# acaelles97/DeVIS

Measured on NVIDIA B200. Metric: temporal_msda_fwd_bwd_layer_clips_per_sec, higher is better.
Workload: dtype f32

## Files before the change

### devis_b200/csrc/msda_bwd.cuh

```cuda
#pragma once
#include "msda_common.cuh"

#ifndef DEVIS_BWD_MIN_BLOCKS
#define DEVIS_BWD_MIN_BLOCKS 3
#endif

namespace devis {

template <class SlotSrc>
struct BwdArgs {
    const void *value;
    const void *grad_out;
    void *grad_value;
    DetScale det;
    Segment seg[2];
    int n_seg;
    int n_slots_total;
    SlotSrc src;
    OpDims d;
    const int *q_perm;
};

template <int LPG>
__device__ __forceinline__ void reduce_scatter_taps(float (&d)[LPG][4], int j, float (&r)[4])
{
#pragma unroll
    for (int half = LPG / 2; half >= 1; half >>= 1) {
        const bool upper = (j & half) != 0;
#pragma unroll
        for (int t = 0; t < half; ++t) {
#pragma unroll
            for (int c = 0; c < 4; ++c) {
                const float send = upper ? d[t][c] : d[t + half][c];
                const float keep = upper ? d[t + half][c] : d[t][c];
                d[t][c] = keep + __shfl_xor_sync(0xffffffffu, send, half, LPG);
            }
        }
    }
#pragma unroll
    for (int c = 0; c < 4; ++c) r[c] = d[0][c];
}

template <bool BF16, int LPG, int QPG, class SlotSrc, bool HALF_ACC = false>
__global__ void __launch_bounds__(256, DEVIS_BWD_MIN_BLOCKS) msda_bwd_kernel(const BwdArgs<SlotSrc> a)
{
    using X = TapExchange<LPG>;
    extern __shared__ int4 s_slot[];
    const int outer = blockIdx.y;
    build_slots(s_slot, a.src, a.d, outer, a.n_slots_total);
    float *xbuf = reinterpret_cast<float *>(s_slot + a.n_slots_total) + (threadIdx.x >> 5) * (2 * X::kWordsPerWarpBuf);

    const int M = a.d.M, Lq = a.d.Lq;
    const int j = threadIdx.x % LPG;
    const int g = (threadIdx.x & 31) / LPG;
    const int grp = threadIdx.x / LPG;
    const int QC = blockDim.x / LPG;
    const int qchunk = blockIdx.x / M, m = blockIdx.x - qchunk * M;
    const L2Policy pol = make_l2_policy();

    int q[QPG];
    bool qlive[QPG];
    float4 go[QPG];
#pragma unroll
    for (int i = 0; i < QPG; ++i) {
        const int qi = (qchunk * QPG + i) * QC + grp;
        qlive[i] = qi < Lq;
        q[i] = qlive[i] ? (a.q_perm ? a.q_perm[qi] : qi) : 0;
        go[i] = make_float4(0.f, 0.f, 0.f, 0.f);
        if (qlive[i]) {
            const size_t row = ((size_t)outer * Lq + q[i]) * M + m;
            go[i] = BF16 ? ldg_bf16x4(reinterpret_cast<const uint2 *>(a.grad_out) + row * LPG + j)
                         : ld_stream_f4(reinterpret_cast<const float4 *>(a.grad_out) + row * LPG + j, pol);
        }
    }

    constexpr unsigned kQuadBytes = BF16 ? 8u : 16u;
    const unsigned rowbytes = (unsigned)(M * LPG) * kQuadBytes;
    const char *vbase = reinterpret_cast<const char *>(a.value) + (size_t)(m * LPG + j) * kQuadBytes;
    asm volatile("" : "+l"(vbase));
    static_assert(!HALF_ACC || BF16, "bf16 accumulation needs bf16 value");
    constexpr unsigned kGvQuadBytes = HALF_ACC ? 8u : 16u;
    char *gvb = a.grad_value ? reinterpret_cast<char *>(a.grad_value) + (size_t)(m * LPG + j) * kGvQuadBytes : nullptr;
    constexpr unsigned kGvShift = (BF16 && !HALF_ACC) ? 1u : 0u;
    char *detb = a.det.acc ? reinterpret_cast<char *>(a.det.acc) + (size_t)(m * LPG) * 32u + (size_t)j * 8u : nullptr;
    const float det_sh = a.det.acc ? ldexpf(1.f, kDetFracBits - det_exponent(a.det.max_bits)) : 0.f;

    int slot_base = 0, parity = 0;
    for (int sg = 0; sg < a.n_seg; ++sg) {
        const int P = a.seg[sg].P, K = a.seg[sg].n_slots * P, pshift = pow2_shift(P);
        const float *loc = reinterpret_cast<const float *>(a.seg[sg].loc);
        const float *aw = reinterpret_cast<const float *>(a.seg[sg].aw);
        float *gloc = reinterpret_cast<float *>(a.seg[sg].grad_loc);
        float *gaw = reinterpret_cast<float *>(a.seg[sg].grad_aw);
        for (int k0 = 0; k0 < K; k0 += LPG) {
            const int k = k0 + j;
            const bool klive = k < K;
            const int4 sl = s_slot[slot_base + (klive ? div_p(k, P, pshift) : 0)];
#pragma unroll
            for (int i = 0; i < QPG; ++i) {
                const size_t row = ((size_t)outer * Lq + q[i]) * M + m;
                const bool live = klive && qlive[i];
                float2 xy = make_float2(0.f, 0.f);
                float w = 0.f;
                if (live) {
                    xy = ld_stream_f2(reinterpret_cast<const float2 *>(loc + row * K * 2) + k, pol);
                    w = ld_stream_f(aw + row * K + k, pol);
                }
                const TapGeom t = tap_geometry(xy.x, xy.y, sl, live);
                float *buf = xbuf + parity * X::kWordsPerWarpBuf;
                parity ^= 1;
                X::publish(buf, j, g, t, w, rowbytes);
                __syncwarp();

                const float4 gg = go[i];
                float dsum[LPG][4];
#pragma unroll
                for (int jj = 0; jj < LPG; ++jj) {
                    uint4 off;
                    float4 c;
                    X::fetch(buf, jj, g, off, c);
                    float4 v00, v01, v10, v11;
                    if (BF16) {
                        v00 = ldg_bf16x4(reinterpret_cast<const uint2 *>(vbase + off.x));
                        v01 = ldg_bf16x4(reinterpret_cast<const uint2 *>(vbase + off.y));
                        v10 = ldg_bf16x4(reinterpret_cast<const uint2 *>(vbase + off.z));
                        v11 = ldg_bf16x4(reinterpret_cast<const uint2 *>(vbase + off.w));
                    } else {
                        v00 = ldg_f4(reinterpret_cast<const float4 *>(vbase + off.x), pol);
                        v01 = ldg_f4(reinterpret_cast<const float4 *>(vbase + off.y), pol);
                        v10 = ldg_f4(reinterpret_cast<const float4 *>(vbase + off.z), pol);
                        v11 = ldg_f4(reinterpret_cast<const float4 *>(vbase + off.w), pol);
                    }
                    dsum[jj][0] = fmaf(v00.w, gg.w, fmaf(v00.z, gg.z, fmaf(v00.y, gg.y, v00.x * gg.x)));
                    dsum[jj][1] = fmaf(v01.w, gg.w, fmaf(v01.z, gg.z, fmaf(v01.y, gg.y, v01.x * gg.x)));
                    dsum[jj][2] = fmaf(v10.w, gg.w, fmaf(v10.z, gg.z, fmaf(v10.y, gg.y, v10.x * gg.x)));
                    dsum[jj][3] = fmaf(v11.w, gg.w, fmaf(v11.z, gg.z, fmaf(v11.y, gg.y, v11.x * gg.x)));
                    if (detb) {
                        if (c.x != 0.f) det_add4<LPG>(reinterpret_cast<long long *>(detb + ((size_t)off.x << (kGvShift + 1))), det_sh, c.x * gg.x, c.x * gg.y, c.x * gg.z, c.x * gg.w);
                        if (c.y != 0.f) det_add4<LPG>(reinterpret_cast<long long *>(detb + ((size_t)off.y << (kGvShift + 1))), det_sh, c.y * gg.x, c.y * gg.y, c.y * gg.z, c.y * gg.w);
                        if (c.z != 0.f) det_add4<LPG>(reinterpret_cast<long long *>(detb + ((size_t)off.z << (kGvShift + 1))), det_sh, c.z * gg.x, c.z * gg.y, c.z * gg.z, c.z * gg.w);
                        if (c.w != 0.f) det_add4<LPG>(reinterpret_cast<long long *>(detb + ((size_t)off.w << (kGvShift + 1))), det_sh, c.w * gg.x, c.w * gg.y, c.w * gg.z, c.w * gg.w);
                    } else if (gvb) {
                        if (c.x != 0.f) red_add_quad<HALF_ACC>(gvb + ((size_t)off.x << kGvShift), c.x * gg.x, c.x * gg.y, c.x * gg.z, c.x * gg.w, pol);
                        if (c.y != 0.f) red_add_quad<HALF_ACC>(gvb + ((size_t)off.y << kGvShift), c.y * gg.x, c.y * gg.y, c.y * gg.z, c.y * gg.w, pol);
                        if (c.z != 0.f) red_add_quad<HALF_ACC>(gvb + ((size_t)off.z << kGvShift), c.z * gg.x, c.z * gg.y, c.z * gg.z, c.z * gg.w, pol);
                        if (c.w != 0.f) red_add_quad<HALF_ACC>(gvb + ((size_t)off.w << kGvShift), c.w * gg.x, c.w * gg.y, c.w * gg.z, c.w * gg.w, pol);
                    }
                }

                float A[4];
                reduce_scatter_taps<LPG>(dsum, j, A);
                if (live) {
                    const bool hit = t.ok != 0u;
                    const float hh = (t.ok & 1u) ? t.hh : 0.f, lh = (t.ok & 2u) ? t.lh : 0.f;
                    const float hw = (t.ok & 4u) ? t.hw : 0.f, lw = (t.ok & 8u) ? t.lw : 0.f;
                    const float l_in = (t.ok & 4u) ? 1.f : 0.f, r_in = (t.ok & 8u) ? 1.f : 0.f;
                    const float t_in = (t.ok & 1u) ? 1.f : 0.f, b_in = (t.ok & 2u) ? 1.f : 0.f;
                    const float val = hh * (hw * A[0] + lw * A[1]) + lh * (hw * A[2] + lw * A[3]);
                    const float gx = hh * (r_in * A[1] - l_in * A[0]) + lh * (r_in * A[3] - l_in * A[2]);
                    const float gy = hw * (b_in * A[2] - t_in * A[0]) + lw * (b_in * A[3] - t_in * A[1]);
                    st_stream_f(gaw + row * K + k, hit ? val : 0.f, pol);
                    st_stream_f2(reinterpret_cast<float2 *>(gloc + row * K * 2) + k,
                                 hit ? make_float2((float)sl.y * gx * w, (float)sl.x * gy * w) : make_float2(0.f, 0.f), pol);
                }
            }
        }
        slot_base += a.seg[sg].n_slots;
    }
}

}
```

### devis_b200/csrc/msda_common.cuh

```cuda
#pragma once
#include <cuda_bf16.h>
#include <cuda_runtime.h>
#include <stdint.h>

namespace devis {

constexpr int kMaxLevels = 16;
constexpr int kMaxFrameTable = 2048;
constexpr int kMaxSlots = 1024;

struct Segment {
    const void *loc;
    const void *aw;
    void *grad_loc;
    void *grad_aw;
    int n_slots;
    int P;
};

struct DeviceLevels {
    const int64_t *shapes;
    const int64_t *lsi;
};

struct ClipTable {
    int H[kMaxLevels];
    int W[kMaxLevels];
    int lsi[kMaxLevels];
    int L;
    int Wt;
    uint8_t frame[kMaxFrameTable];
};

struct OpDims {
    int outer;
    int S;
    int M, D;
    int Lq;
};

__device__ __forceinline__ void build_slots(int4 *s_slot, const DeviceLevels &lv, const OpDims &d, int outer,
                                            int n_slots)
{
    for (int s = threadIdx.x; s < n_slots; s += blockDim.x) {
        const int H = (int)lv.shapes[2 * s], W = (int)lv.shapes[2 * s + 1];
        s_slot[s] = make_int4(H, W, outer * d.S + (int)lv.lsi[s], W * d.M);
    }
    __syncthreads();
}

__device__ __forceinline__ void build_slots(int4 *s_slot, const ClipTable &tb, const OpDims &d, int outer,
                                            int n_slots)
{
    for (int s = threadIdx.x; s < n_slots; s += blockDim.x) {
        int frame, l;
        if (s < tb.L) {
            frame = outer;
            l = s;
        } else {
            const int j = (s - tb.L) / tb.L;
            l = (s - tb.L) - j * tb.L;
            frame = tb.frame[outer * tb.Wt + j];
        }
        s_slot[s] = make_int4(tb.H[l], tb.W[l], frame * d.S + tb.lsi[l], tb.W[l] * d.M);
    }
    __syncthreads();
}

__device__ __forceinline__ int pow2_shift(int v) { return (v > 0 && (v & (v - 1)) == 0) ? __ffs(v) - 1 : -1; }
__device__ __forceinline__ int div_p(int k, int P, int pshift) { return pshift >= 0 ? (k >> pshift) : (k / P); }
__device__ __forceinline__ int mod_l(int s, int L, int lshift) { return lshift >= 0 ? (s & (L - 1)) : (s % L); }

struct TapGeom {
    float lh, lw, hh, hw;
    int rTL, rTR, rBL, rBR;
    int y0c, x0c;
    unsigned ok;
};

__device__ __forceinline__ TapGeom tap_geometry(float x, float y, const int4 slot, bool live)
{
    TapGeom g;
    const int H = slot.x, W = slot.y;
    const float h_im = __fadd_rn(__fmul_rn(y, (float)H), -0.5f);
    const float w_im = __fadd_rn(__fmul_rn(x, (float)W), -0.5f);
    const bool inb = live && h_im > -1.f && w_im > -1.f && h_im < (float)H && w_im < (float)W;
    const float hf = floorf(h_im), wf = floorf(w_im);
    const int h0 = inb ? (int)hf : 0, w0 = inb ? (int)wf : 0;
    g.lh = h_im - hf;
    g.lw = w_im - wf;
    g.hh = 1.f - g.lh;
    g.hw = 1.f - g.lw;
    g.ok = inb ? ((unsigned)(h0 >= 0) | ((unsigned)(h0 + 1 <= H - 1) << 1) | ((unsigned)(w0 >= 0) << 2) |
                  ((unsigned)(w0 + 1 <= W - 1) << 3))
               : 0u;
    const int h0c = max(h0, 0), h1c = min(h0 + 1, H - 1), w0c = max(w0, 0), w1c = min(w0 + 1, W - 1);
    const int top = slot.z + h0c * W, bot = slot.z + h1c * W;
    g.y0c = h0c;
    g.x0c = w0c;
    g.rTL = top + w0c;
    g.rTR = top + w1c;
    g.rBL = bot + w0c;
    g.rBR = bot + w1c;
    return g;
}

struct TapGeomV {
    float lh, lw, hh, hw;
    int rowv;
    unsigned live;
    unsigned ok;
};

__device__ __forceinline__ TapGeomV tap_geometry_v(float x, float y, const int4 slot, bool live)
{
    TapGeomV g;
    const int H = slot.x, W = slot.y;
    const float h_im = __fadd_rn(__fmul_rn(y, (float)H), -0.5f);
    const float w_im = __fadd_rn(__fmul_rn(x, (float)W), -0.5f);
    const bool inb = live && h_im > -1.f && w_im > -1.f && h_im < (float)H && w_im < (float)W;
    const float hf = floorf(h_im), wf = floorf(w_im);
    const int h0 = inb ? (int)hf : 0, w0 = inb ? (int)wf : 0;
    g.lh = h_im - hf;
    g.lw = w_im - wf;
    g.hh = 1.f - g.lh;
    g.hw = 1.f - g.lw;
    const unsigned top = h0 >= 0, bot = h0 + 1 <= H - 1, left = w0 >= 0, right = w0 + 1 <= W - 1;
    g.ok = inb ? (top | (bot << 1) | (left << 2) | (right << 3)) : 0u;
    g.live = inb ? ((top & left) | ((top & right) << 1) | ((bot & left) << 2) | ((bot & right) << 3)) : 0u;
    g.rowv = slot.z + h0 * W + w0;
    return g;
}

template <int LPG>
struct TapExchange {
    static constexpr int GPW = 32 / LPG;
    static constexpr int kWordsPerWarpBuf = LPG * GPW * 8;
    static constexpr int kBytesPerWarp = 2 * kWordsPerWarpBuf * 4;

    __device__ static __forceinline__ int rec_word(int j, int g) { return (j * GPW + (g ^ (j & (GPW - 1)))) * 8; }

    __device__ static __forceinline__ void publish(float *buf, int j, int g, const TapGeom &t, float w, unsigned rowbytes,
                                                   unsigned tag = 0u)
    {
        const bool live = t.ok != 0u;
        uint4 off;
        off.x = ((unsigned)t.rTL * rowbytes) | tag;
        off.y = (unsigned)t.rTR * rowbytes;
        off.z = (unsigned)t.rBL * rowbytes;
        off.w = (unsigned)t.rBR * rowbytes;
        float4 f;
        f.x = (live && (t.ok & 1u)) ? w * t.hh : 0.f;
        f.y = (live && (t.ok & 2u)) ? w * t.lh : 0.f;
        f.z = (t.ok & 4u) ? t.hw : 0.f;
        f.w = (t.ok & 8u) ? t.lw : 0.f;
        float *r = buf + rec_word(j, g);
        if (j & 4) {
            *reinterpret_cast<float4 *>(r + 4) = f;
            *reinterpret_cast<uint4 *>(r) = off;
        } else {
            *reinterpret_cast<uint4 *>(r) = off;
            *reinterpret_cast<float4 *>(r + 4) = f;
        }
    }

    __device__ static __forceinline__ void fetch(const float *buf, int jj, int g, uint4 &off, float4 &c)
    {
        const float *r = buf + rec_word(jj, g);
        off = *reinterpret_cast<const uint4 *>(r);
        const float4 f = *reinterpret_cast<const float4 *>(r + 4);
        c.x = f.x * f.z;
        c.y = f.x * f.w;
        c.z = f.y * f.z;
        c.w = f.y * f.w;
    }
};

#ifndef DEVIS_HINTS
#define DEVIS_HINTS 7
#endif

__device__ __forceinline__ float2 ld_stream_f2(const float2 *p)
{
#if DEVIS_HINTS & 1
    float2 v;
    asm("ld.global.nc.L1::no_allocate.v2.f32 {%0,%1}, [%2];" : "=f"(v.x), "=f"(v.y) : "l"(p));
    return v;
#else
    return __ldg(p);
#endif
}

__device__ __forceinline__ float ld_stream_f(const float *p)
{
#if DEVIS_HINTS & 1
    float v;
    asm("ld.global.nc.L1::no_allocate.f32 %0, [%1];" : "=f"(v) : "l"(p));
    return v;
#else
    return __ldg(p);
#endif
}

__device__ __forceinline__ void st_stream_f4(float4 *p, float4 v)
{
#if DEVIS_HINTS & 2
    asm volatile("st.global.L1::no_allocate.v4.f32 [%0], {%1,%2,%3,%4};" ::"l"(p), "f"(v.x), "f"(v.y), "f"(v.z), "f"(v.w) : "memory");
#else
    *p = v;
#endif
}

__device__ __forceinline__ void st_stream_f2(float2 *p, float2 v)
{
#if DEVIS_HINTS & 2
    asm volatile("st.global.L1::no_allocate.v2.f32 [%0], {%1,%2};" ::"l"(p), "f"(v.x), "f"(v.y) : "memory");
#else
    *p = v;
#endif
}

__device__ __forceinline__ void st_stream_f(float *p, float v)
{
#if DEVIS_HINTS & 2
    asm volatile("st.global.L1::no_allocate.f32 [%0], %1;" ::"l"(p), "f"(v) : "memory");
#else
    *p = v;
#endif
}

#ifndef DEVIS_L2_HINTS
#define DEVIS_L2_HINTS 0
#endif

struct L2Policy {
    unsigned long long stream;
    unsigned long long keep;
};

__device__ __forceinline__ L2Policy make_l2_policy()
{
    L2Policy p;
    p.stream = 0ull;
    p.keep = 0ull;
#if DEVIS_L2_HINTS & 1
    asm("createpolicy.fractional.L2::evict_first.b64 %0, 1.0;" : "=l"(p.stream));
#endif
#if DEVIS_L2_HINTS & 6
    asm("createpolicy.fractional.L2::evict_last.b64 %0, 1.0;" : "=l"(p.keep));
#endif
    return p;
}

__device__ __forceinline__ float2 ld_stream_f2(const float2 *p, const L2Policy &pol)
{
#if DEVIS_L2_HINTS & 1
    float2 v;
    asm("ld.global.nc.L1::no_allocate.L2::cache_hint.v2.f32 {%0,%1}, [%2], %3;" : "=f"(v.x), "=f"(v.y) : "l"(p), "l"(pol.stream));
    return v;
#else
    return ld_stream_f2(p);
#endif
}

__device__ __forceinline__ float ld_stream_f(const float *p, const L2Policy &pol)
{
#if DEVIS_L2_HINTS & 1
    float v;
    asm("ld.global.nc.L1::no_allocate.L2::cache_hint.f32 %0, [%1], %2;" : "=f"(v) : "l"(p), "l"(pol.stream));
    return v;
#else
    return ld_stream_f(p);
#endif
}

__device__ __forceinline__ float4 ld_stream_f4(const float4 *p, const L2Policy &pol)
{
#if DEVIS_L2_HINTS & 1
    float4 v;
    asm("ld.global.nc.L1::no_allocate.L2::cache_hint.v4.f32 {%0,%1,%2,%3}, [%4], %5;"
        : "=f"(v.x), "=f"(v.y), "=f"(v.z), "=f"(v.w) : "l"(p), "l"(pol.stream));
    return v;
#else
    return __ldg(p);
#endif
}

__device__ __forceinline__ void st_stream_f4(float4 *p, float4 v, const L2Policy &pol)
{
#if DEVIS_L2_HINTS & 1
    asm volatile("st.global.L1::no_allocate.L2::cache_hint.v4.f32 [%0], {%1,%2,%3,%4}, %5;" ::"l"(p), "f"(v.x), "f"(v.y),
                 "f"(v.z), "f"(v.w), "l"(pol.stream) : "memory");
#else
    st_stream_f4(p, v);
#endif
}

__device__ __forceinline__ void st_stream_f2(float2 *p, float2 v, const L2Policy &pol)
{
#if DEVIS_L2_HINTS & 1
    asm volatile("st.global.L1::no_allocate.L2::cache_hint.v2.f32 [%0], {%1,%2}, %3;" ::"l"(p), "f"(v.x), "f"(v.y),
                 "l"(pol.stream) : "memory");
#else
    st_stream_f2(p, v);
#endif
}

__device__ __forceinline__ void st_stream_f(float *p, float v, const L2Policy &pol)
{
#if DEVIS_L2_HINTS & 1
    asm volatile("st.global.L1::no_allocate.L2::cache_hint.f32 [%0], %1, %2;" ::"l"(p), "f"(v), "l"(pol.stream) : "memory");
#else
    st_stream_f(p, v);
#endif
}

__device__ __forceinline__ float4 ldg_f4(const float4 *p)
{
#if DEVIS_HINTS & 4
    float4 v;
    asm("ld.global.nc.L1::evict_last.v4.f32 {%0,%1,%2,%3}, [%4];" : "=f"(v.x), "=f"(v.y), "=f"(v.z), "=f"(v.w) : "l"(p));
    return v;
#else
    return __ldg(p);
#endif
}

__device__ __forceinline__ float4 ldg_f4(const float4 *p, const L2Policy &pol)
{
#if DEVIS_L2_HINTS & 2
    float4 v;
    asm("ld.global.nc.L1::evict_last.L2::cache_hint.v4.f32 {%0,%1,%2,%3}, [%4], %5;"
        : "=f"(v.x), "=f"(v.y), "=f"(v.z), "=f"(v.w) : "l"(p), "l"(pol.keep));
    return v;
#else
    return ldg_f4(p);
#endif
}

__device__ __forceinline__ float4 ldg_bf16x4(const uint2 *p)
{
    const uint2 r = __ldg(p);
    float4 o;
    o.x = __uint_as_float(r.x << 16);
    o.y = __uint_as_float(r.x & 0xffff0000u);
    o.z = __uint_as_float(r.y << 16);
    o.w = __uint_as_float(r.y & 0xffff0000u);
    return o;
}

__device__ __forceinline__ void red_add_f4(float *p, float a, float b, float c, float d)
{
    asm volatile("red.global.add.v4.f32 [%0], {%1,%2,%3,%4};" ::"l"(p), "f"(a), "f"(b), "f"(c), "f"(d) : "memory");
}

__device__ __forceinline__ void red_add_bf16x4(void *p, float a, float b, float c, float d)
{
    const __nv_bfloat162 lo = __floats2bfloat162_rn(a, b), hi = __floats2bfloat162_rn(c, d);
    asm volatile("red.global.add.noftz.v2.bf16x2 [%0], {%1,%2};" ::"l"(p),
                 "r"(*reinterpret_cast<const unsigned *>(&lo)), "r"(*reinterpret_cast<const unsigned *>(&hi))
                 : "memory");
}

__device__ __forceinline__ void red_add_f4(float *p, float a, float b, float c, float d, const L2Policy &pol)
{
#if DEVIS_L2_HINTS & 4
    asm volatile("red.global.add.L2::cache_hint.v4.f32 [%0], {%1,%2,%3,%4}, %5;" ::"l"(p), "f"(a), "f"(b), "f"(c), "f"(d),
                 "l"(pol.keep) : "memory");
#else
    red_add_f4(p, a, b, c, d);
#endif
}

template <bool HALF>
__device__ __forceinline__ void red_add_quad(char *p, float a, float b, float c, float d)
{
    if (HALF) red_add_bf16x4(p, a, b, c, d);
    else red_add_f4(reinterpret_cast<float *>(p), a, b, c, d);
}

template <bool HALF>
__device__ __forceinline__ void red_add_quad(char *p, float a, float b, float c, float d, const L2Policy &pol)
{
    if (HALF) red_add_bf16x4(p, a, b, c, d);
    else red_add_f4(reinterpret_cast<float *>(p), a, b, c, d, pol);
}

struct DetScale {
    const unsigned *max_bits;
    long long *acc;
};

constexpr int kDetFracBits = 36;

__device__ __forceinline__ int det_exponent(const unsigned *max_bits, int n_factors = 2)
{
    float bound = __uint_as_float(max_bits[0]);
    for (int i = 1; i < n_factors; ++i) bound *= __uint_as_float(max_bits[i]);
    int e = 0;
    if (bound > 0.f && bound < 3.0e38f) (void)frexpf(bound, &e);
    return e + 1;
}

template <int LPG>
__device__ __forceinline__ void det_add4(long long *p, float sh, float a, float b, float c, float d)
{
    atomicAdd(reinterpret_cast<unsigned long long *>(p) + 0 * LPG, (unsigned long long)__float2ll_rn(a * sh));
    atomicAdd(reinterpret_cast<unsigned long long *>(p) + 1 * LPG, (unsigned long long)__float2ll_rn(b * sh));
    atomicAdd(reinterpret_cast<unsigned long long *>(p) + 2 * LPG, (unsigned long long)__float2ll_rn(c * sh));
    atomicAdd(reinterpret_cast<unsigned long long *>(p) + 3 * LPG, (unsigned long long)__float2ll_rn(d * sh));
}

template <bool BF16>
__global__ void __launch_bounds__(256) absmax_kernel(const void *x, size_t n, unsigned *slot)
{
    float m = 0.f;
    for (size_t i = (size_t)blockIdx.x * blockDim.x + threadIdx.x; i < n; i += (size_t)gridDim.x * blockDim.x) {
        const float v = BF16 ? __bfloat162float(reinterpret_cast<const __nv_bfloat16 *>(x)[i])
                             : reinterpret_cast<const float *>(x)[i];
        m = fmaxf(m, fabsf(v));
    }
#pragma unroll
    for (int o = 16; o >= 1; o >>= 1) m = fmaxf(m, __shfl_xor_sync(0xffffffffu, m, o));
    if ((threadIdx.x & 31) == 0) atomicMax(slot, __float_as_uint(m));
}

static __global__ void set_word_kernel(unsigned *slot, unsigned bits) { *slot = bits; }

static __global__ void __launch_bounds__(256) det_finalize_kernel(const long long *acc, float *out, size_t n,
                                                           const unsigned *max_bits, int lpg, int n_factors = 2)
{
    const double back = ldexp(1.0, det_exponent(max_bits, n_factors) - kDetFracBits);
    for (size_t i = (size_t)blockIdx.x * blockDim.x + threadIdx.x; i < n; i += (size_t)gridDim.x * blockDim.x) {
        size_t src = i;
        if (lpg) {
            const int ch = (int)(i % (size_t)(4 * lpg));
            src = i - ch + (size_t)((ch & 3) * lpg + (ch >> 2));
        }
        out[i] = (float)((double)acc[src] * back);
    }
}

__device__ __forceinline__ uint2 pack_bf16x4(float4 v)
{
    const __nv_bfloat162 lo = __floats2bfloat162_rn(v.x, v.y), hi = __floats2bfloat162_rn(v.z, v.w);
    uint2 r;
    r.x = *reinterpret_cast<const unsigned *>(&lo);
    r.y = *reinterpret_cast<const unsigned *>(&hi);
    return r;
}

}
```

Measured before the change: 524.3.

## Merge duplicate bilinear corners across neighbouring taps before grad_value atomics

```diff
diff --git a/devis_b200/csrc/msda_bwd.cuh b/devis_b200/csrc/msda_bwd.cuh
--- a/devis_b200/csrc/msda_bwd.cuh
+++ b/devis_b200/csrc/msda_bwd.cuh
@@ -41,6 +41,42 @@
     for (int c = 0; c < 4; ++c) r[c] = d[0][c];
 }
 
+template <int LPG>
+__device__ __forceinline__ float4 merge_slot_duplicates(const float4 c, int rowv, int W, int j, int k0, int K, int P,
+                                                        int pshift)
+{
+    const float mine[4] = {c.x, c.y, c.z, c.w};
+    float sum[4] = {c.x, c.y, c.z, c.w};
+    unsigned absorbed = 0u;
+    const int k = k0 + j;
+    const int s = div_p(k < K ? k : 0, P, pshift);
+#pragma unroll
+    for (int x = 1; x < 4 && x < LPG; ++x) {
+        const int rb = __shfl_xor_sync(0xffffffffu, rowv, x, LPG);
+        const int kb = k0 + (j ^ x);
+        const int d = rb - rowv;
+        const int ddy = d >= W - 1 ? 1 : (d <= 1 - W ? -1 : 0);
+        const int ddx = d - ddy * W;
+        const bool near = W >= 3 && k < K && kb < K && div_p(kb, P, pshift) == s && ddx >= -1 && ddx <= 1;
+        const bool earlier = (j ^ x) < j;
+#pragma unroll
+        for (int qb = 0; qb < 4; ++qb) {
+            const float cb = __shfl_xor_sync(0xffffffffu, mine[qb], x, LPG);
+            const int qy = (qb >> 1) + ddy, qx = (qb & 1) + ddx;
+            const bool on = near && cb != 0.f && qy >= 0 && qy <= 1 && qx >= 0 && qx <= 1;
+            const int q = (qy << 1) | qx;
+#pragma unroll
+            for (int u = 0; u < 4; ++u) {
+                const bool hit = on && q == u && mine[u] != 0.f;
+                absorbed |= (hit && earlier) ? 1u << u : 0u;
+                sum[u] += (hit && !earlier) ? cb : 0.f;
+            }
+        }
+    }
+    return make_float4((absorbed & 1u) ? 0.f : sum[0], (absorbed & 2u) ? 0.f : sum[1], (absorbed & 4u) ? 0.f : sum[2],
+                       (absorbed & 8u) ? 0.f : sum[3]);
+}
+
 template <bool BF16, int LPG, int QPG, class SlotSrc, bool HALF_ACC = false>
 __global__ void __launch_bounds__(256, DEVIS_BWD_MIN_BLOCKS) msda_bwd_kernel(const BwdArgs<SlotSrc> a)
 {
@@ -109,7 +145,12 @@
                 const TapGeom t = tap_geometry(xy.x, xy.y, sl, live);
                 float *buf = xbuf + parity * X::kWordsPerWarpBuf;
                 parity ^= 1;
-                X::publish(buf, j, g, t, w, rowbytes);
+                float4 coef = X::corner_coefs(t, w);
+#ifndef DEVIS_BWD_MERGE
+#define DEVIS_BWD_MERGE 1
+#endif
+                if (DEVIS_BWD_MERGE && !detb) coef = merge_slot_duplicates<LPG>(coef, t.rowv, sl.y, j, k0, K, P, pshift);
+                X::publish_corners(buf, j, g, t, coef, rowbytes);
                 __syncwarp();
 
                 const float4 gg = go[i];
@@ -118,7 +159,7 @@
                 for (int jj = 0; jj < LPG; ++jj) {
                     uint4 off;
                     float4 c;
-                    X::fetch(buf, jj, g, off, c);
+                    X::fetch_corners(buf, jj, g, off, c);
                     float4 v00, v01, v10, v11;
                     if (BF16) {
                         v00 = ldg_bf16x4(reinterpret_cast<const uint2 *>(vbase + off.x));
diff --git a/devis_b200/csrc/msda_common.cuh b/devis_b200/csrc/msda_common.cuh
--- a/devis_b200/csrc/msda_common.cuh
+++ b/devis_b200/csrc/msda_common.cuh
@@ -75,6 +75,7 @@
     float lh, lw, hh, hw;
     int rTL, rTR, rBL, rBR;
     int y0c, x0c;
+    int rowv;
     unsigned ok;
 };
 
@@ -98,6 +99,7 @@
     const int top = slot.z + h0c * W, bot = slot.z + h1c * W;
     g.y0c = h0c;
     g.x0c = w0c;
+    g.rowv = slot.z + h0 * W + w0;
     g.rTL = top + w0c;
     g.rTR = top + w1c;
     g.rBL = bot + w0c;
@@ -174,6 +176,39 @@
         c.z = f.y * f.z;
         c.w = f.y * f.w;
     }
+
+    __device__ static __forceinline__ float4 corner_coefs(const TapGeom &t, float w)
+    {
+        const bool live = t.ok != 0u;
+        const float fx = (live && (t.ok & 1u)) ? w * t.hh : 0.f, fy = (live && (t.ok & 2u)) ? w * t.lh : 0.f;
+        const float fz = (t.ok & 4u) ? t.hw : 0.f, fw = (t.ok & 8u) ? t.lw : 0.f;
+        return make_float4(fx * fz, fx * fw, fy * fz, fy * fw);
+    }
+
+    __device__ static __forceinline__ void publish_corners(float *buf, int j, int g, const TapGeom &t, float4 c,
+                                                           unsigned rowbytes)
+    {
+        uint4 off;
+        off.x = (unsigned)t.rTL * rowbytes;
+        off.y = (unsigned)t.rTR * rowbytes;
+        off.z = (unsigned)t.rBL * rowbytes;
+        off.w = (unsigned)t.rBR * rowbytes;
+        float *r = buf + rec_word(j, g);
+        if (j & 4) {
+            *reinterpret_cast<float4 *>(r + 4) = c;
+            *reinterpret_cast<uint4 *>(r) = off;
+        } else {
+            *reinterpret_cast<uint4 *>(r) = off;
+            *reinterpret_cast<float4 *>(r + 4) = c;
+        }
+    }
+
+    __device__ static __forceinline__ void fetch_corners(const float *buf, int jj, int g, uint4 &off, float4 &c)
+    {
+        const float *r = buf + rec_word(jj, g);
+        off = *reinterpret_cast<const uint4 *>(r);
+        c = *reinterpret_cast<const float4 *>(r + 4);
+    }
 };
 
 #ifndef DEVIS_HINTS
```

After: 497.5, median of 6. 0.949x the previous value.
